# cmusphinx/pocketsphinx

Hardware: NVIDIA H100
Metric: frames/sec senone-eval+Viterbi (higher is better)
Workload: dtype f32->i16/i32

## Files before the change

### pocketsphinx_b200/csrc/psb_hmm.cu

```cuda
#include "psb_hmmctx.cuh"

#include <stdlib.h>
#include <string.h>

#include <algorithm>
#include <type_traits>

#include <vector>


struct psb_phoneloop_s {
    psb_hmmctx_t *c;
    int n_phones, window, beam, pbeam, pip;
    double penalty_weight;
    Stream stream;
    DevBuf<int32_t> d_ssid, d_tmatid;
    DevBuf<uint16_t> d_senid;
};

namespace {

__device__ __forceinline__ void load_hmm(const psb_hmm_t *p, HmmReg &h, int n)
{
#pragma unroll
// ... 283 lines not shown
        if (rc) return rc;
    }
    int rc = ensure_hmm_cap(c, n);
    if (rc) return rc;
    memcpy(c->h_hmms, hmms, (size_t)n * sizeof(psb_hmm_t));
    rc = eval_staged(c, n, senscr, best);
    if (rc) return rc;
    for (int i = 0; i < n; ++i) {
        void *ctx = hmms[i].ctx;
        hmms[i] = c->h_hmms[i];
        hmms[i].ctx = ctx;
    }
    return PSB_OK;
}

extern "C" int psb_hmm_vit_eval_ptrs(psb_hmmctx_t *c, psb_hmm_t *const *hmms, int32_t n, const int16_t *senscr,
                                     int32_t *best)
{
    PSB_REQUIRE(c && n >= 0 && (n == 0 || (hmms && senscr)), "psb_hmm_vit_eval_ptrs: bad argument");
    if (best) *best = PSB_WORST_SCORE;
    if (n == 0) return PSB_OK;
    PSB_CUDA(cudaSetDevice(c->device));
    int rc = ensure_hmm_cap(c, n);
    if (rc) return rc;
    for (int i = 0; i < n; ++i) {
        PSB_REQUIRE(hmms[i], "hmms[%d] is null", i);
        rc = validate_hmm(c, hmms[i], i);
        if (rc) return rc;
        c->h_hmms[i] = *hmms[i];
    }
    rc = eval_staged(c, n, senscr, best);
    if (rc) return rc;
    for (int i = 0; i < n; ++i) {
        void *ctx = hmms[i]->ctx;
        *hmms[i] = c->h_hmms[i];
        hmms[i]->ctx = ctx;
    }
    return PSB_OK;
}


extern "C" int psb_phoneloop_create(psb_hmmctx_t *c, int32_t n_phones, const int32_t *ssid, const int32_t *tmatid,
                                    int32_t window, int32_t beam, int32_t pbeam, int32_t pip, double penalty_weight,
                                    psb_phoneloop_t **out)
{
    PSB_REQUIRE(c && out && n_phones > 0 && ssid && tmatid && window >= 0, "psb_phoneloop_create: bad argument");
    PSB_CUDA(cudaSetDevice(c->device));
    std::vector<uint16_t> senid((size_t)c->n_emit * n_phones);
    int rc = ctx_senids(c, "psb_phoneloop_create", n_phones, ssid, tmatid, senid.data(), 1, n_phones);
    if (rc) return rc;
    std::unique_ptr<psb_phoneloop_t> p(new psb_phoneloop_t());
    p->c = c; p->n_phones = n_phones; p->window = window; p->beam = beam; p->pbeam = pbeam; p->pip = pip;
    p->penalty_weight = penalty_weight;
    rc = p->d_senid.reserve(senid.size());
    if (!rc) rc = p->d_tmatid.reserve((size_t)n_phones);
    if (!rc) rc = p->d_ssid.reserve((size_t)n_phones);
    if (rc) return rc;
    cudaError_t e = cudaMemcpy(p->d_senid, senid.data(), senid.size() * 2, cudaMemcpyHostToDevice);
    if (e == cudaSuccess) e = cudaMemcpy(p->d_tmatid, tmatid, (size_t)n_phones * 4, cudaMemcpyHostToDevice);
    if (e == cudaSuccess) e = cudaMemcpy(p->d_ssid, ssid, (size_t)n_phones * 4, cudaMemcpyHostToDevice);
    if (e == cudaSuccess) e = p->stream.create();
    if (e != cudaSuccess) {
        psb_set_error("psb_phoneloop_create: %s", cudaGetErrorString(e));
        return PSB_ERR_CUDA;
    }
    *out = p.release();
    return PSB_OK;
}

extern "C" void psb_phoneloop_free(psb_phoneloop_t *p)
{
    if (!p) return;
    cudaSetDevice(p->c->device);
    cudaStreamSynchronize(p->stream);
    delete p;
}

int psb_phoneloop_launch(psb_phoneloop_t *p, const int16_t *d_senscr, const int32_t *d_utt_off, int32_t n_utt,
                         int32_t *d_best, int32_t *d_pen, psb_hmm_t *d_final, psb_hmm_t *d_trace, cudaStream_t st)
{
    const int H = p->n_phones, N = p->c->n_emit;
    size_t smem = ((size_t)(2 * N + 4 + p->window) * H + 64) * sizeof(int);
    PSB_REQUIRE(smem <= 227 * 1024, "phone loop with %d HMMs needs %zu bytes of shared memory (max 227 KB)", H, smem);
    PSB_CUDA(cudaFuncSetAttribute(phoneloop_kernel, cudaFuncAttributeMaxDynamicSharedMemorySize, (int)smem));
    int threads = std::min(1024, roundup(H, 32));
    PlParams P;
    P.n_phones = H; P.window = p->window; P.beam = p->beam; P.pbeam = p->pbeam; P.pip = p->pip;
    P.penalty_weight = p->penalty_weight;
    phoneloop_kernel<<<n_utt, threads, smem, st>>>(d_senscr, d_utt_off, dev_ctx(p->c), P, p->d_senid, p->d_tmatid, p->d_ssid,
                                                   d_best, d_pen, d_final, d_trace);
    PSB_LAUNCH_CHECK();
    return PSB_OK;
}

int psb_phoneloop_n_phones(const psb_phoneloop_t *p) { return p->n_phones; }

extern "C" int psb_phoneloop_run_device(psb_phoneloop_t *p, const int16_t *d_senscr, const int32_t *utt_off,
                                        int32_t n_utt, int32_t *d_best, int32_t *d_pen, psb_hmm_t *final_hmms,
                                        void *batch)
{
    PSB_REQUIRE(p && d_senscr && utt_off && n_utt >= 0, "psb_phoneloop_run_device: bad argument");
    if (n_utt == 0) return PSB_OK;
    int rc = ctx_check_utts("psb_phoneloop_run_device", utt_off, n_utt, d_senscr);
    if (rc) return rc;
    PSB_CUDA(cudaSetDevice(p->c->device));
    cudaStream_t st = batch ? psb_batch_stream((psb_batch_t *)batch) : p->stream;
    DevBuf<int32_t> d_off;
    DevBuf<psb_hmm_t> d_final;
    if ((rc = d_off.reserve((size_t)n_utt + 1))) return rc;
    if (final_hmms && (rc = d_final.reserve((size_t)n_utt * p->n_phones))) return rc;
    PSB_CUDA(cudaMemcpyAsync(d_off, utt_off, (size_t)(n_utt + 1) * 4, cudaMemcpyHostToDevice, st));
    rc = psb_phoneloop_launch(p, d_senscr, d_off, n_utt, d_best, d_pen, d_final, nullptr, st);
    if (!rc && final_hmms) {
        cudaError_t e = cudaMemcpyAsync(final_hmms, d_final, (size_t)n_utt * p->n_phones * sizeof(psb_hmm_t),
                                        cudaMemcpyDeviceToHost, st);
        if (e != cudaSuccess) { psb_set_error("%s", cudaGetErrorString(e)); rc = PSB_ERR_CUDA; }
    }
    cudaStreamSynchronize(st);
    return rc;
}

extern "C" int psb_phoneloop_run_host(psb_phoneloop_t *p, const int16_t *senscr, const int32_t *utt_off, int32_t n_utt,
                                      int32_t *best, int32_t *pen, psb_hmm_t *hmm_trace)
{
    PSB_REQUIRE(p && senscr && utt_off && n_utt >= 0, "psb_phoneloop_run_host: bad argument");
    if (n_utt == 0) return PSB_OK;
    int rc = ctx_check_utts("psb_phoneloop_run_host", utt_off, n_utt, senscr);
    if (rc) return rc;
    PSB_CUDA(cudaSetDevice(p->c->device));
    const size_t total = utt_off[n_utt], H = p->n_phones;
    DevBuf<int16_t> d_scr;
    DevBuf<int32_t> d_off, d_best, d_pen;
    DevBuf<psb_hmm_t> d_tr;
    if ((rc = d_scr.reserve(std::max<size_t>(1, total * p->c->n_sen))) || (rc = d_off.reserve((size_t)n_utt + 1)) ||
        (best && (rc = d_best.reserve(std::max<size_t>(1, total)))) || (pen && (rc = d_pen.reserve(std::max<size_t>(1, total * H)))) ||
        (hmm_trace && (rc = d_tr.reserve(std::max<size_t>(1, total * H)))))
        return rc;
    cudaError_t e = cudaMemcpy(d_scr, senscr, total * p->c->n_sen * 2, cudaMemcpyHostToDevice);
    if (e == cudaSuccess) e = cudaMemcpy(d_off, utt_off, (size_t)(n_utt + 1) * 4, cudaMemcpyHostToDevice);
    if (e == cudaSuccess) {
        rc = psb_phoneloop_launch(p, d_scr, d_off, n_utt, d_best, d_pen, nullptr, d_tr, p->stream);
        if (!rc) e = cudaStreamSynchronize(p->stream);
        if (!rc && e == cudaSuccess && best) e = cudaMemcpy(best, d_best, total * 4, cudaMemcpyDeviceToHost);
        if (!rc && e == cudaSuccess && pen) e = cudaMemcpy(pen, d_pen, total * H * 4, cudaMemcpyDeviceToHost);
        if (!rc && e == cudaSuccess && hmm_trace)
            e = cudaMemcpy(hmm_trace, d_tr, total * H * sizeof(psb_hmm_t), cudaMemcpyDeviceToHost);
    }
    if (e != cudaSuccess) { psb_set_error("psb_phoneloop_run_host: %s", cudaGetErrorString(e)); rc = PSB_ERR_CUDA; }
    return rc;
}

constexpr int HS_V = 4;
constexpr int HS_TS = 512;
constexpr int SWEEP_FR = 4;
constexpr int HS_THREADS = 128;

struct psb_hmmset_s {
    psb_hmmctx_t *c;
    int64_t n_max, n, pitch;
    int32_t n_seg_max, n_seg;
    int64_t max_seg_len;
    bool any_mpx;
    Stream own_stream;
    cudaStream_t stream;
    DevBuf<int32_t> d_i32;
    DevBuf<uint16_t> d_u16;
    DevBuf<uint8_t> d_mpx;
    DevBuf<int64_t> d_seg_off;
    DevBuf<int64_t> d_seg_base;
    DevBuf<psb_hmm_t> d_aos;
    DevBuf<int32_t> d_snap_i32;
    Event ev[2];
};

namespace {

struct HmmSetDev {
    int32_t *i32;
    uint16_t *u16;
    uint8_t *mpx;
    const int64_t *seg_off, *seg_base;
    int64_t pitch;
    int n_seg;
};

static HmmSetDev dev_set(const psb_hmmset_t *s)
{
    HmmSetDev d;
    d.i32 = s->d_i32; d.u16 = s->d_u16; d.mpx = s->d_mpx; d.seg_off = s->d_seg_off; d.seg_base = s->d_seg_base;
    d.pitch = s->pitch; d.n_seg = s->n_seg;
    return d;
}

template <bool TO_SOA>
__global__ void __launch_bounds__(256)
hmmset_convert_kernel(psb_hmm_t *aos, HmmSetDev s, int64_t n, int ns)
{
    const int64_t a = (int64_t)blockIdx.x * blockDim.x + threadIdx.x;
    if (a >= n) return;
    int lo = 0, hi = s.n_seg;
    while (hi - lo > 1) {
        const int mid = (lo + hi) >> 1;
        if (s.seg_off[mid] <= a) lo = mid; else hi = mid;
    }
    const int64_t i = s.seg_base[lo] + (a - s.seg_off[lo]);
    psb_hmm_t *p = aos + a;
    const int64_t b32 = (i / HS_TS) * (int64_t)(2 * ns + 4) * HS_TS + (i % HS_TS);
    const int64_t b16 = (i / HS_TS) * (int64_t)(ns + 2) * HS_TS + (i % HS_TS);
    int32_t *score = s.i32 + b32, *hist = score + ns * HS_TS, *tail = score + 2 * ns * HS_TS;
    uint16_t *senid = s.u16 + b16, *ids = senid + ns * HS_TS;
    if (TO_SOA) {
        for (int k = 0; k < ns; ++k) {
            score[k * HS_TS] = p->score[k];
            hist[k * HS_TS] = p->history[k];
            senid[k * HS_TS] = p->senid[k];
        }
        tail[0] = p->out_score; tail[HS_TS] = p->out_history; tail[2 * HS_TS] = p->bestscore; tail[3 * HS_TS] = p->frame;
        ids[0] = p->ssid; ids[HS_TS] = (uint16_t)p->tmatid;
        s.mpx[i] = p->mpx;
    }
    else {
        for (int k = 0; k < PSB_HMM_MAX_NSTATE; ++k) {
            p->score[k] = k < ns ? score[k * HS_TS] : 0;
            p->history[k] = k < ns ? hist[k * HS_TS] : 0;
            p->senid[k] = k < ns ? senid[k * HS_TS] : 0;
        }
        p->out_score = tail[0]; p->out_history = tail[HS_TS]; p->bestscore = tail[2 * HS_TS]; p->frame = tail[3 * HS_TS];
        p->ssid = ids[0]; p->tmatid = (int16_t)ids[HS_TS];
        p->mpx = s.mpx[i]; p->n_emit_state = (uint8_t)ns;
        p->ctx = nullptr;
    }
}

__global__ void fill_i32_kernel(int32_t *p, int64_t n, int32_t v)
{
    const int64_t i = (int64_t)blockIdx.x * blockDim.x + threadIdx.x;
    if (i < n) p[i] = v;
}

__device__ __forceinline__ int comp(const int4 &v, int q) { return q == 0 ? v.x : q == 1 ? v.y : q == 2 ? v.z : v.w; }
__device__ __forceinline__ void setc(int4 &v, int q, int x)
{
    if (q == 0) v.x = x; else if (q == 1) v.y = x; else if (q == 2) v.z = x; else v.w = x;
}

__device__ __forceinline__ void mbar_init(uint64_t *bar, int count)
{
    asm volatile("mbarrier.init.shared::cta.b64 [%0], %1;" ::"r"((unsigned)__cvta_generic_to_shared(bar)), "r"(count));
}
__device__ __forceinline__ void mbar_expect_tx(uint64_t *bar, unsigned bytes)
{
    asm volatile("mbarrier.arrive.expect_tx.shared::cta.b64 _, [%0], %1;" ::"r"((unsigned)__cvta_generic_to_shared(bar)), "r"(bytes)
                 : "memory");
}
__device__ __forceinline__ void mbar_wait(uint64_t *bar, unsigned parity)
{
    asm volatile(
        "{\n"
        ".reg .pred p;\n"
        "WAIT_%=:\n"
        "mbarrier.try_wait.parity.shared::cta.b64 p, [%0], %1;\n"
        "@p bra DONE_%=;\n"
        "bra WAIT_%=;\n"
        "DONE_%=:\n"
        "}\n" ::"r"((unsigned)__cvta_generic_to_shared(bar)),
        "r"(parity)
        : "memory");
}
__device__ __forceinline__ void tma_bulk_g2s(void *dst, const void *src, unsigned bytes, uint64_t *bar)
{
    asm volatile("cp.async.bulk.shared::cluster.global.mbarrier::complete_tx::bytes [%0], [%1], %2, [%3];" ::"r"(
                     (unsigned)__cvta_generic_to_shared(dst)),
                 "l"(src), "r"(bytes), "r"((unsigned)__cvta_generic_to_shared(bar))
                 : "memory");
}

template <int NS>
__global__ void __launch_bounds__(HS_THREADS, NS == 3 ? 6 : 4)
hmmset_eval_kernel(HmmSetDev s, HmmCtxDev c, const int16_t *__restrict__ senscr, const int64_t *__restrict__ row0,
                   const int32_t *__restrict__ n_rows, int t, int32_t *__restrict__ best_out)
{
    extern __shared__ __align__(16) int16_t srow[];
    __shared__ int red[HS_THREADS / 32];
    const int seg = blockIdx.y;
    if (n_rows && t >= n_rows[seg]) return;
    const int64_t n = s.seg_off[seg + 1] - s.seg_off[seg];
    const int64_t j0 = ((int64_t)blockIdx.x * HS_THREADS + threadIdx.x) * HS_V;
    if ((int64_t)blockIdx.x * HS_THREADS * HS_V >= n) return;
    constexpr int NL = NS > 0 ? NS : PSB_HMM_MAX_NSTATE;
    const int ns = NS > 0 ? NS : c.n_emit;
    const bool live = j0 < n;
    const int64_t i = s.seg_base[seg] + (live ? j0 : 0);
    const int64_t b32 = (i / HS_TS) * (int64_t)(2 * ns + 4) * HS_TS + (i % HS_TS);
    const int64_t b16 = (i / HS_TS) * (int64_t)(ns + 2) * HS_TS + (i % HS_TS);
    int32_t *score = s.i32 + b32, *hist = score + ns * HS_TS, *tail = score + 2 * ns * HS_TS;
    uint16_t *senid = s.u16 + b16;
    const uint16_t *ids = senid + ns * HS_TS;
    int4 sc[NL], hi[NL], osc, ohi, bst;
    uint2 sid[NL], tm = make_uint2(0u, 0u);
    uchar4 mp = make_uchar4(0, 0, 0, 0);
    if (live) {
#pragma unroll
        for (int k = 0; k < NL; ++k)
            if (k < ns) {
                sc[k] = __ldcs(reinterpret_cast<const int4 *>(score + k * HS_TS));
                hi[k] = __ldcs(reinterpret_cast<const int4 *>(hist + k * HS_TS));
                sid[k] = __ldcs(reinterpret_cast<const uint2 *>(senid + k * HS_TS));
            }
        osc = __ldcs(reinterpret_cast<const int4 *>(tail));
        ohi = __ldcs(reinterpret_cast<const int4 *>(tail + HS_TS));
        tm = __ldcs(reinterpret_cast<const uint2 *>(ids + HS_TS));
        mp = __ldcs(reinterpret_cast<const uchar4 *>(s.mpx + i));
    }
    __shared__ __align__(8) uint64_t row_bar;
    const int16_t *srow_al;
    {
        const int16_t *row = senscr + (row0 ? row0[seg] + t : (int64_t)t * gridDim.y + seg) * c.n_sen;
        const uintptr_t a = reinterpret_cast<uintptr_t>(row);
        const unsigned mis = (unsigned)(a & 15), nbytes = (unsigned)c.n_sen * 2;
        unsigned head = (16 - mis) & 15;
        if (head > nbytes) head = nbytes;
        const unsigned body = (nbytes - head) & ~15u, tail = nbytes - head - body;
        unsigned char *dst = reinterpret_cast<unsigned char *>(srow) + mis;
        if (threadIdx.x == 0) {
            mbar_init(&row_bar, 1);
            asm volatile("fence.mbarrier_init.release.cluster;" ::: "memory");
            if (body) {
                mbar_expect_tx(&row_bar, body);
                tma_bulk_g2s(dst + head, reinterpret_cast<const unsigned char *>(row) + head, body, &row_bar);
            }
        }
        const unsigned hn = head >> 1, tn = tail >> 1;
        if (threadIdx.x < hn) reinterpret_cast<int16_t *>(dst)[threadIdx.x] = row[threadIdx.x];
        if (threadIdx.x >= 32 && threadIdx.x < 32 + tn)
            reinterpret_cast<int16_t *>(dst + head + body)[threadIdx.x - 32] = row[((head + body) >> 1) + threadIdx.x - 32];
        srow_al = reinterpret_cast<const int16_t *>(dst);
        __syncthreads();
        if (body) mbar_wait(&row_bar, 0u);
    }
    int best = PSB_WORST_SCORE;
    if (live) {
        bool any_mpx = false;
#pragma unroll
        for (int q = 0; q < HS_V; ++q) {
            HmmReg h;
#pragma unroll
            for (int k = 0; k < PSB_HMM_MAX_NSTATE; ++k) {
                const bool in = k < NL && k < ns;
                h.score[k] = in ? comp(sc[k < NL ? k : 0], q) : PSB_WORST_SCORE;
                h.hist[k] = in ? comp(hi[k < NL ? k : 0], q) : -1;
                const unsigned w = (q < 2) ? sid[k < NL ? k : 0].x : sid[k < NL ? k : 0].y;
                h.senid[k] = in ? (int)((q & 1) ? (w >> 16) : (w & 0xffffu)) : PSB_BAD_SSID;
            }
            h.out_score = comp(osc, q);
            h.out_hist = comp(ohi, q);
            h.best = PSB_WORST_SCORE;
            const unsigned tw = (q < 2) ? tm.x : tm.y;
            const int tmatid = (int16_t)((q & 1) ? (tw >> 16) : (tw & 0xffffu));
// ... 194 lines not shown
            if (NS == 3) {
                int (&s3)[3] = *reinterpret_cast<int (*)[3]>(sc[v]);
                int (&h3)[3] = *reinterpret_cast<int (*)[3]>(hi[v]);
                bb = hmm_step_3st_dec<decltype(s1_known)::value>(s3, h3, osc[v], ohi[v], tk[v], score_at(sid[v][0]), score_at(sid[v][1]),
                                      score_at(sid[v][NS > 2 ? 2 : 0]));
            }
            else {
                HmmReg h;
                int obs[PSB_HMM_MAX_NSTATE];
#pragma unroll
                for (int k = 0; k < PSB_HMM_MAX_NSTATE; ++k) {
                    h.score[k] = k < NS ? sc[v][k < NS ? k : 0] : PSB_WORST_SCORE;
                    h.hist[k] = k < NS ? hi[v][k < NS ? k : 0] : -1;
                    h.senid[k] = 0;
                    obs[k] = k < NS ? -score_at(sid[v][k < NS ? k : 0]) : 0;
                }
                h.out_score = osc[v]; h.out_hist = ohi[v]; h.best = PSB_WORST_SCORE;
                bb = hmm_step_5st(h, tps + tmo[v], obs);
#pragma unroll
                for (int k = 0; k < NS; ++k) { sc[v][k] = h.score[k]; hi[v][k] = h.hist[k]; }
                osc[v] = h.out_score; ohi[v] = h.out_hist;
            }
            if (!LIVE_TEST || v * THREADS < rem) best = max(best, bb);
            best_final[v] = bb;
        }
        };
        if (NS == 3 && FAST && s1_live) frame_steps(std::true_type());
        else frame_steps(std::false_type());
        best = __reduce_max_sync(0xffffffffu, best);
        if (BEAM) cnt = __reduce_add_sync(0xffffffffu, cnt);
        const int slot = t % (2 * FR);
        if ((tid & 31) == 0) {
            red[slot][tid >> 5] = best;
            if (BEAM) redc[b][tid >> 5] = cnt;
        }
        if (FR > 1 && t % FR != FR - 1 && t + 1 < T) continue;
        const int tf = t - t % FR;
        __syncthreads();
        if (tid == 0 && !cta_empty)
#pragma unroll 1
            for (int u = tf + NBUF; u <= t + NBUF; ++u)
                if (u < T && tma_ok(u)) issue(u);
        if (tid < 32) {
            if (!BEAM) {
#pragma unroll 1
                for (int u = tf; u <= t; ++u) {
                    int v = tid < THREADS / 32 ? red[u % (2 * FR)][tid] : PSB_WORST_SCORE;
                    v = __reduce_max_sync(0xffffffffu, v);
                    if (tid == 0) atomicMax(best_out + (size_t)u * gridDim.y + seg, v);
                }
            }
            else {
                int v = tid < THREADS / 32 ? red[slot][tid] : PSB_WORST_SCORE;
                v = __reduce_max_sync(0xffffffffu, v);
                int cc = tid < THREADS / 32 ? redc[b][tid] : 0;
                cc = __reduce_add_sync(0xffffffffu, cc);
                if (tid == 0) mbar_expect_tx(&xbar[b], n_rank * 8u);
                if ((unsigned)tid < n_rank)
                    st_async_v2(mapa_shared(&cl_slot[b][my_rank], (unsigned)tid), (unsigned)v, (unsigned)cc,
                                mapa_shared(&xbar[b], (unsigned)tid));
            }
        }
        if (BEAM) {
            mbar_wait(&xbar[b], (unsigned)(t >> 1) & 1u);
            int seg_best = PSB_WORST_SCORE, seg_cnt = 0;
            for (unsigned r = 0; r < n_rank; ++r) {
                const int2 m = cl_slot[b][r];
                seg_best = max(seg_best, m.x);
                seg_cnt += m.y;
            }
            if (my_rank == 0 && tid == 0) {
                best_out[(size_t)t * gridDim.y + seg] = seg_best;
                if (n_active_out) n_active_out[(size_t)t * gridDim.y + seg] = seg_cnt;
            }
            hist[b ^ 1][tid] = 0u;
            int dyn = beam;
            if (maxhmmpf >= 0 && seg_cnt > maxhmmpf) {
                const int bw = -beam / 256;
#pragma unroll
                for (int v = 0; v < V; ++v)
                    if (act[v]) {
                        int bin = (seg_best - best_final[v]) / bw;
                        bin = bin > 255 ? 255 : bin;
                        atomicAdd(&hist[b][bin], 1u);
                    }
                if (tid == 0) found = 256;
                cluster_sync_all();
                unsigned tot = 0;
                for (unsigned r = 0; r < n_rank; ++r) tot += ld_cluster_u32(mapa_shared(&hist[b][tid], r));
                unsigned incl = tot;
#pragma unroll
                for (int o = 1; o < 32; o <<= 1) {
                    const unsigned y = __shfl_up_sync(0xffffffffu, incl, o);
                    if ((tid & 31) >= o) incl += y;
                }
                if ((tid & 31) == 31) scan_w[tid >> 5] = incl;
                __syncthreads();
                for (int w = 0; w < (tid >> 5); ++w) incl += scan_w[w];
                if (incl > (unsigned)maxhmmpf) atomicMin(&found, tid);
                __syncthreads();
                dyn = -(found * bw);
            }
            const int thresh = seg_best + dyn;
#pragma unroll
            for (int v = 0; v < V; ++v)
                if (act[v] && !(best_final[v] > thresh)) {
#pragma unroll
                    for (int k = 0; k < NS; ++k) { sc[v][k] = PSB_WORST_SCORE; hi[v][k] = -1; }
                    osc[v] = PSB_WORST_SCORE; ohi[v] = -1; best_final[v] = PSB_WORST_SCORE;
                    act[v] = false;
                }
        }
    }
    if (BEAM) cluster_sync_all();
#pragma unroll
    for (int v = 0; v < V; ++v) {
        if (!live[v] || !touched[v]) continue;
        int32_t *p32 = state_i32(v);
#pragma unroll
        for (int k = 0; k < NS; ++k) {
            p32[k * HS_TS] = sc[v][k];
            p32[(NS + k) * HS_TS] = hi[v][k];
        }
        p32[2 * NS * HS_TS] = osc[v];
        p32[(2 * NS + 1) * HS_TS] = ohi[v];
        p32[(2 * NS + 2) * HS_TS] = best_final[v];
        if (BEAM) p32[(2 * NS + 3) * HS_TS] = act[v] ? frame0 + T : -1;
    }
}

}

extern "C" void psb_hmmset_free(psb_hmmset_t *s)
{
    if (!s) return;
    cudaSetDevice(s->c->device);
    if (s->stream) cudaStreamSynchronize(s->stream);
    delete s;
}

extern "C" int psb_hmmset_create(psb_hmmctx_t *c, int64_t n_max, int32_t n_seg_max, psb_hmmset_t **out)
{
    PSB_REQUIRE(c && out && n_max > 0 && n_seg_max > 0 && n_seg_max <= 65535, "psb_hmmset_create: bad argument");
    const char *v = getenv("PSB_HMMSET_THREADS");
    PSB_REQUIRE(!v || !strcmp(v, "128"), "psb_hmmset_create: PSB_HMMSET_THREADS=%s; the only accepted value is 128", v);
    PSB_CUDA(cudaSetDevice(c->device));
    std::unique_ptr<psb_hmmset_t> s(new psb_hmmset_t());
    s->c = c; s->n_max = n_max; s->n_seg_max = n_seg_max;
    s->pitch = ((n_max + (int64_t)(HS_V - 1) * n_seg_max + HS_TS - 1) / HS_TS) * HS_TS;
    const int ns = c->n_emit;
    int rc = s->d_i32.reserve((size_t)(2 * ns + 4) * s->pitch);
    if (!rc) rc = s->d_u16.reserve((size_t)(ns + 2) * s->pitch);
    if (!rc) rc = s->d_mpx.reserve((size_t)s->pitch);
    if (!rc) rc = s->d_seg_off.reserve((size_t)n_seg_max + 1);
    if (!rc) rc = s->d_seg_base.reserve((size_t)n_seg_max + 1);
    if (rc) return rc;
    cudaError_t e = s->own_stream.create();
    s->stream = s->own_stream;
    if (e == cudaSuccess) e = s->ev[0].create();
    if (e == cudaSuccess) e = s->ev[1].create();
    if (e != cudaSuccess) {
        psb_set_error("psb_hmmset_create: %s", cudaGetErrorString(e));
        return PSB_ERR_CUDA;
    }
    *out = s.release();
    return PSB_OK;
}

extern "C" int psb_hmmset_use_batch_stream(psb_hmmset_t *s, psb_batch_t *b)
{
    PSB_REQUIRE(s, "psb_hmmset_use_batch_stream: null set");
    PSB_CUDA(cudaStreamSynchronize(s->stream));
    s->stream = b ? psb_batch_stream(b) : s->own_stream;
    return PSB_OK;
}

extern "C" int psb_hmmset_snapshot(psb_hmmset_t *s)
{
    PSB_REQUIRE(s && !s->any_mpx, "psb_hmmset_snapshot: null set or multiplexed instances");
    PSB_CUDA(cudaSetDevice(s->c->device));
    const size_t nb = (size_t)(2 * s->c->n_emit + 4) * s->pitch * 4;
    const int rc = s->d_snap_i32.reserve(nb / 4);
    if (rc) return rc;
    PSB_CUDA(cudaMemcpyAsync(s->d_snap_i32, s->d_i32, nb, cudaMemcpyDeviceToDevice, s->stream));
    return PSB_OK;
}

extern "C" int psb_hmmset_restore(psb_hmmset_t *s)
{
    PSB_REQUIRE(s && s->d_snap_i32, "psb_hmmset_restore: no snapshot");
    PSB_CUDA(cudaSetDevice(s->c->device));
    PSB_CUDA(cudaMemcpyAsync(s->d_i32, s->d_snap_i32, (size_t)(2 * s->c->n_emit + 4) * s->pitch * 4, cudaMemcpyDeviceToDevice, s->stream));
    return PSB_OK;
}

static int hmmset_staging(psb_hmmset_t *s)
{
    return s->d_aos.reserve((size_t)s->n_max);
}

extern "C" int psb_hmmset_upload(psb_hmmset_t *s, const psb_hmm_t *hmms, int64_t n, const int64_t *seg_off, int32_t n_seg)
{
    PSB_REQUIRE(s && n >= 0 && n <= s->n_max && n_seg > 0 && n_seg <= s->n_seg_max && seg_off && (n == 0 || hmms),
                "psb_hmmset_upload: bad argument");
    PSB_REQUIRE(seg_off[0] == 0 && seg_off[n_seg] == n, "psb_hmmset_upload: seg_off must run from 0 to n");
    PSB_CUDA(cudaSetDevice(s->c->device));
    int64_t mx = 0;
    std::vector<int64_t> base((size_t)n_seg + 1);
    base[0] = 0;
    for (int pass = 0; pass < 2; ++pass) {
        const int big = pass == 0 ? HS_TS : HS_V;
        for (int i = 0; i < n_seg; ++i) {
            PSB_REQUIRE(seg_off[i + 1] >= seg_off[i], "psb_hmmset_upload: seg_off not monotone at %d", i);
            const int64_t len = seg_off[i + 1] - seg_off[i];
            const int pad = len >= HS_TS ? big : HS_V;
            mx = std::max<int64_t>(mx, len);
            base[(size_t)i + 1] = base[(size_t)i] + (len + pad - 1) / pad * pad;
        }
        if (base[(size_t)n_seg] <= s->pitch) break;
    }
    PSB_REQUIRE(base[(size_t)n_seg] <= s->pitch, "psb_hmmset_upload: internal capacity exceeded");
    s->any_mpx = false;
    for (int64_t i = 0; i < n; ++i) {
        int rc = validate_hmm(s->c, &hmms[i], (int)i);
        if (rc) return rc;
        s->any_mpx |= hmms[i].mpx != 0;
    }
    int rc = hmmset_staging(s);
    if (rc) return rc;
    s->n = n; s->n_seg = n_seg; s->max_seg_len = mx;
    PSB_CUDA(cudaMemcpyAsync(s->d_seg_off, seg_off, (size_t)(n_seg + 1) * 8, cudaMemcpyHostToDevice, s->stream));
    PSB_CUDA(cudaMemcpyAsync(s->d_seg_base, base.data(), (size_t)(n_seg + 1) * 8, cudaMemcpyHostToDevice, s->stream));
    const int ns = s->c->n_emit;
    const int64_t ni = (int64_t)(2 * ns + 4) * s->pitch;
    fill_i32_kernel<<<(unsigned)((ni + 255) / 256), 256, 0, s->stream>>>(s->d_i32, ni, PSB_WORST_SCORE);
    PSB_LAUNCH_CHECK();
    PSB_CUDA(cudaMemsetAsync(s->d_u16, 0, (size_t)(ns + 2) * s->pitch * 2, s->stream));
    PSB_CUDA(cudaMemsetAsync(s->d_mpx, 0, (size_t)s->pitch, s->stream));
    if (n) {
        PSB_CUDA(cudaMemcpyAsync(s->d_aos, hmms, (size_t)n * sizeof(psb_hmm_t), cudaMemcpyHostToDevice, s->stream));
        hmmset_convert_kernel<true><<<(unsigned)((n + 255) / 256), 256, 0, s->stream>>>(s->d_aos, dev_set(s), n, ns);
        PSB_LAUNCH_CHECK();
    }
    PSB_CUDA(cudaStreamSynchronize(s->stream));
    return PSB_OK;
}

extern "C" int psb_hmmset_download(psb_hmmset_t *s, psb_hmm_t *hmms)
{
    PSB_REQUIRE(s && (s->n == 0 || hmms), "psb_hmmset_download: bad argument");
    if (s->n == 0) return PSB_OK;
    PSB_CUDA(cudaSetDevice(s->c->device));
    int rc = hmmset_staging(s);
    if (rc) return rc;
    hmmset_convert_kernel<false><<<(unsigned)((s->n + 255) / 256), 256, 0, s->stream>>>(s->d_aos, dev_set(s), s->n, s->c->n_emit);
    PSB_LAUNCH_CHECK();
    std::vector<psb_hmm_t> tmp((size_t)s->n);
    PSB_CUDA(cudaMemcpyAsync(tmp.data(), s->d_aos, (size_t)s->n * sizeof(psb_hmm_t), cudaMemcpyDeviceToHost, s->stream));
    PSB_CUDA(cudaStreamSynchronize(s->stream));
    for (int64_t i = 0; i < s->n; ++i) {
        void *ctx = hmms[i].ctx;
        hmms[i] = tmp[(size_t)i];
        hmms[i].ctx = ctx;
    }
    return PSB_OK;
}

extern "C" int psb_hmmset_eval_frames_device(psb_hmmset_t *s, const int16_t *d_senscr, const int64_t *d_row0,
                                             const int32_t *d_n_rows, int32_t n_frames, int32_t *d_best, float *ms)
{
    PSB_REQUIRE(s && d_senscr && d_best && n_frames >= 0, "psb_hmmset_eval_frames_device: bad argument");
    if (ms) *ms = 0.f;
    if (n_frames == 0 || s->n_seg == 0) return PSB_OK;
    PSB_CUDA(cudaSetDevice(s->c->device));
    const int64_t nb = (int64_t)n_frames * s->n_seg;
    fill_i32_kernel<<<(unsigned)((nb + 255) / 256), 256, 0, s->stream>>>(d_best, nb, PSB_WORST_SCORE);
    PSB_LAUNCH_CHECK();
    if (s->n == 0) {
        PSB_CUDA(cudaStreamSynchronize(s->stream));
        return PSB_OK;
    }
    const int tile = HS_THREADS * HS_V;
    const dim3 grid((unsigned)((s->max_seg_len + tile - 1) / tile), (unsigned)s->n_seg);
    const HmmSetDev sd = dev_set(s);
    const HmmCtxDev cd = dev_ctx(s->c);
    const size_t smem = (((size_t)cd.n_sen * 2 + 15) & ~(size_t)15) + 16;
    PSB_REQUIRE(smem <= 200 * 1024, "psb_hmmset: %d senones do not fit the shared-memory score row", cd.n_sen);
    auto launch = [&](auto kern, int t, int32_t *best) {
        kern<<<grid, HS_THREADS, smem, s->stream>>>(sd, cd, d_senscr, d_row0, d_n_rows, t, best);
    };
#define PSB_HS_ATTR(NS) PSB_CUDA(cudaFuncSetAttribute(hmmset_eval_kernel<NS>, cudaFuncAttributeMaxDynamicSharedMemorySize, (int)smem))
    if (smem > 48 * 1024) {
        PSB_HS_ATTR(3); PSB_HS_ATTR(5); PSB_HS_ATTR(0);
    }
#undef PSB_HS_ATTR
    PSB_CUDA(cudaEventRecord(s->ev[0], s->stream));
    for (int t = 0; t < n_frames; ++t) {
        int32_t *best = d_best + (size_t)t * s->n_seg;
        if (cd.n_emit == 3) launch(hmmset_eval_kernel<3>, t, best);
        else if (cd.n_emit == 5) launch(hmmset_eval_kernel<5>, t, best);
        else launch(hmmset_eval_kernel<0>, t, best);
        PSB_LAUNCH_CHECK();
    }
    PSB_CUDA(cudaEventRecord(s->ev[1], s->stream));
    PSB_CUDA(cudaStreamSynchronize(s->stream));
    if (ms) PSB_CUDA(cudaEventElapsedTime(ms, s->ev[0], s->ev[1]));
    return PSB_OK;
}

template <int NS, int V, int THREADS, int FR, bool LIVE_TEST = (NS != 3), bool FAST = (NS == 3)>
static int sweep_launch(psb_hmmset_t *s, const int16_t *d_senscr, int64_t rows_total, const int64_t *d_row0,
                        const int32_t *d_n_rows, int32_t n_frames, int32_t *d_best)
{
    const HmmCtxDev cd = dev_ctx(s->c);
    const int buf_bytes = (int)(((size_t)cd.n_sen * 2 + 32 + 127) & ~(size_t)127);
    const int tp_bytes = s->c->n_tmat * NS * (NS + 1);
    const size_t smem = 2 * FR * (size_t)buf_bytes + tp_bytes;
    PSB_REQUIRE(smem <= 200 * 1024, "psb_hmmset_sweep: %d senones / %d transition matrices do not fit shared memory", cd.n_sen, s->c->n_tmat);
    auto kern = hmmset_sweep_kernel<NS, V, THREADS, false, FR, LIVE_TEST, FAST>;
    PSB_CUDA(cudaFuncSetAttribute(kern, cudaFuncAttributeMaxDynamicSharedMemorySize, (int)smem));
    const dim3 grid((unsigned)((s->max_seg_len + THREADS * V - 1) / (THREADS * V)), (unsigned)s->n_seg);
    PSB_CUDA(cudaEventRecord(s->ev[0], s->stream));
    kern<<<grid, THREADS, smem, s->stream>>>(dev_set(s), cd, d_senscr, (long long)rows_total, d_row0, d_n_rows, n_frames, d_best,
                                            s->c->n_tmat, buf_bytes, 0, 0, -1, nullptr);
    PSB_LAUNCH_CHECK();
    PSB_CUDA(cudaEventRecord(s->ev[1], s->stream));
    return PSB_OK;
}

static int sweep_device(psb_hmmset_t *s, const int16_t *d_senscr, int64_t rows_total, const int64_t *d_row0,
                        const int32_t *d_n_rows, int32_t n_frames, int32_t *d_best, int candidate, float *ms)
{
    PSB_REQUIRE(s && d_senscr && d_best && n_frames >= 0 && rows_total > 0, "psb_hmmset_sweep_device: bad argument");
    const HmmCtxDev cd = dev_ctx(s->c);
    if (s->any_mpx || (cd.n_emit != 3 && cd.n_emit != 5) || (cd.n_sen & 1))
        return psb_hmmset_eval_frames_device(s, d_senscr, d_row0, d_n_rows, n_frames, d_best, ms);
    if (ms) *ms = 0.f;
    if (n_frames == 0 || s->n_seg == 0) return PSB_OK;
    PSB_CUDA(cudaSetDevice(s->c->device));
    const int64_t nb = (int64_t)n_frames * s->n_seg;
    fill_i32_kernel<<<(unsigned)((nb + 255) / 256), 256, 0, s->stream>>>(d_best, nb, PSB_WORST_SCORE);
    PSB_LAUNCH_CHECK();
    if (s->n == 0) {
        if (ms) PSB_CUDA(cudaStreamSynchronize(s->stream));
        return PSB_OK;
    }
    int rc;
    if (cd.n_emit == 5) rc = sweep_launch<5, 4, 512, SWEEP_FR>(s, d_senscr, rows_total, d_row0, d_n_rows, n_frames, d_best);
#ifdef PSB_SWEEP_CANDIDATES
    else if (candidate == 1) rc = sweep_launch<3, 4, 256, 2>(s, d_senscr, rows_total, d_row0, d_n_rows, n_frames, d_best);
    else if (candidate == 2) rc = sweep_launch<3, 4, 512, 1>(s, d_senscr, rows_total, d_row0, d_n_rows, n_frames, d_best);
    else if (candidate == 3) rc = sweep_launch<3, 4, 512, 4, false, false>(s, d_senscr, rows_total, d_row0, d_n_rows, n_frames, d_best);
    else if (candidate == 4) rc = sweep_launch<3, 4, 512, 8>(s, d_senscr, rows_total, d_row0, d_n_rows, n_frames, d_best);
    else if (candidate == 5) rc = sweep_launch<3, 4, 256, 2, true, false>(s, d_senscr, rows_total, d_row0, d_n_rows, n_frames, d_best);
    else if (candidate == 6) rc = sweep_launch<3, 4, 512, 2, true, false>(s, d_senscr, rows_total, d_row0, d_n_rows, n_frames, d_best);
    else if (candidate == 7) rc = sweep_launch<3, 4, 512, 2>(s, d_senscr, rows_total, d_row0, d_n_rows, n_frames, d_best);
    else if (candidate == 8) rc = sweep_launch<3, 4, 256, 4>(s, d_senscr, rows_total, d_row0, d_n_rows, n_frames, d_best);
#endif
    else rc = sweep_launch<3, 4, 512, SWEEP_FR>(s, d_senscr, rows_total, d_row0, d_n_rows, n_frames, d_best);
    (void)candidate;
    if (rc) return rc;
    if (ms) {
        PSB_CUDA(cudaStreamSynchronize(s->stream));
        PSB_CUDA(cudaEventElapsedTime(ms, s->ev[0], s->ev[1]));
    }
    return PSB_OK;
}

extern "C" int psb_hmmset_sweep_device(psb_hmmset_t *s, const int16_t *d_senscr, int64_t rows_total, const int64_t *d_row0,
                                       const int32_t *d_n_rows, int32_t n_frames, int32_t *d_best, float *ms)
{
    return sweep_device(s, d_senscr, rows_total, d_row0, d_n_rows, n_frames, d_best, 0, ms);
}

#ifdef PSB_SWEEP_CANDIDATES
extern "C" int psb_hmmset_sweep_candidate_device(psb_hmmset_t *s, const int16_t *d_senscr, int64_t rows_total, const int64_t *d_row0,
                                                 const int32_t *d_n_rows, int32_t n_frames, int32_t *d_best, int32_t candidate,
                                                 float *ms)
{
    return sweep_device(s, d_senscr, rows_total, d_row0, d_n_rows, n_frames, d_best, candidate, ms);
}
#endif

extern "C" int psb_hmmset_sweep_beam_device(psb_hmmset_t *s, const int16_t *d_senscr, int64_t rows_total, const int64_t *d_row0,
                                            const int32_t *d_n_rows, int32_t n_frames, int32_t frame0, int32_t beam,
                                            int32_t maxhmmpf, int32_t *d_best, int32_t *d_n_active, float *ms)
{
    PSB_REQUIRE(s && d_senscr && d_best && n_frames >= 0 && rows_total > 0, "psb_hmmset_sweep_beam_device: bad argument");
    PSB_REQUIRE(beam < 0 && beam > -0x20000000, "psb_hmmset_sweep_beam_device: the beam is a negative log score (got %d)", beam);
    PSB_REQUIRE(maxhmmpf < 0 || beam <= -256, "psb_hmmset_sweep_beam_device: -maxhmmpf needs a beam of at least 256 score units (bin width -beam/256)");
    const HmmCtxDev cd = dev_ctx(s->c);
    PSB_REQUIRE(!s->any_mpx && (cd.n_emit == 3 || cd.n_emit == 5) && !(cd.n_sen & 1),
                "psb_hmmset_sweep_beam_device: plain 3- or 5-state instances and an even senone count (the fused kernel's shapes)");
    constexpr int THREADS = 256, V = 4;
    const int64_t per_seg = (s->max_seg_len + THREADS * V - 1) / (THREADS * V);
    PSB_REQUIRE(per_seg <= 16, "psb_hmmset_sweep_beam_device: a segment of %lld instances needs %lld CTAs, a cluster holds 16",
                (long long)s->max_seg_len, (long long)per_seg);
    if (ms) *ms = 0.f;
    if (n_frames == 0 || s->n_seg == 0) return PSB_OK;
    PSB_CUDA(cudaSetDevice(s->c->device));
    const int64_t nb = (int64_t)n_frames * s->n_seg;
    fill_i32_kernel<<<(unsigned)((nb + 255) / 256), 256, 0, s->stream>>>(d_best, nb, PSB_WORST_SCORE);
    PSB_LAUNCH_CHECK();
    if (d_n_active) PSB_CUDA(cudaMemsetAsync(d_n_active, 0, (size_t)nb * 4, s->stream));
    if (s->n == 0) {
        if (ms) PSB_CUDA(cudaStreamSynchronize(s->stream));
        return PSB_OK;
    }
    const int buf_bytes = (int)(((size_t)cd.n_sen * 2 + 32 + 127) & ~(size_t)127);
    const int tp_bytes = s->c->n_tmat * cd.n_emit * (cd.n_emit + 1);
    const size_t smem = 6 * (size_t)buf_bytes + tp_bytes;
    PSB_REQUIRE(smem <= 200 * 1024, "psb_hmmset_sweep_beam: %d senones / %d transition matrices do not fit shared memory", cd.n_sen, s->c->n_tmat);
    const HmmSetDev sd = dev_set(s);
    const long long rows_ll = rows_total;
    const int n_tmat = s->c->n_tmat;
    cudaLaunchConfig_t cfg = {};
    cfg.gridDim = dim3((unsigned)std::max<int64_t>(per_seg, 1), (unsigned)s->n_seg);
    cfg.blockDim = dim3(THREADS);
    cfg.dynamicSmemBytes = smem;
    cfg.stream = s->stream;
    cudaLaunchAttribute at[1];
    at[0].id = cudaLaunchAttributeClusterDimension;
    at[0].val.clusterDim.x = cfg.gridDim.x; at[0].val.clusterDim.y = 1; at[0].val.clusterDim.z = 1;
    cfg.attrs = at; cfg.numAttrs = 1;
    PSB_CUDA(cudaEventRecord(s->ev[0], s->stream));
#define PSB_SWEEPB(NS)                                                                                                         \
    do {                                                                                                                       \
        auto kern = hmmset_sweep_kernel<NS, V, THREADS, true>;                                                                 \
        PSB_CUDA(cudaFuncSetAttribute(kern, cudaFuncAttributeMaxDynamicSharedMemorySize, (int)smem));                          \
        if (cfg.gridDim.x > 8) PSB_CUDA(cudaFuncSetAttribute(kern, cudaFuncAttributeNonPortableClusterSizeAllowed, 1));       \
        int n_clusters = 0;                                                                                                    \
        PSB_CUDA(cudaOccupancyMaxActiveClusters(&n_clusters, kern, &cfg));                                                     \
        PSB_REQUIRE(n_clusters > 0, "psb_hmmset_sweep_beam: a cluster of %u CTAs with %zu bytes of shared memory each does not fit the device", \
                    cfg.gridDim.x, smem);                                                                                      \
        PSB_CUDA(cudaLaunchKernelEx(&cfg, kern, sd, cd, d_senscr, rows_ll, d_row0, d_n_rows, (int)n_frames, d_best, n_tmat,   \
                                    buf_bytes, (int)frame0, (int)beam, (int)maxhmmpf, d_n_active));                            \
        PSB_LAUNCH_CHECK();                                                                                                    \
    } while (0)
    if (cd.n_emit == 3) PSB_SWEEPB(3);
    else PSB_SWEEPB(5);
#undef PSB_SWEEPB
    PSB_CUDA(cudaEventRecord(s->ev[1], s->stream));
    if (ms) {
        PSB_CUDA(cudaStreamSynchronize(s->stream));
        PSB_CUDA(cudaEventElapsedTime(ms, s->ev[0], s->ev[1]));
    }
    return PSB_OK;
}

extern "C" int psb_hmmset_eval_host(psb_hmmset_t *s, const int16_t *senscr, int32_t *best)
{
    PSB_REQUIRE(s && senscr && best, "psb_hmmset_eval_host: bad argument");
    PSB_CUDA(cudaSetDevice(s->c->device));
    DevBuf<int16_t> d_scr;
    DevBuf<int32_t> d_best;
    const size_t nb = (size_t)s->n_seg * s->c->n_sen * 2;
    int rc = d_scr.reserve(nb / 2);
    if (!rc) rc = d_best.reserve((size_t)s->n_seg);
    if (rc) return rc;
    cudaError_t e = cudaMemcpy(d_scr, senscr, nb, cudaMemcpyHostToDevice);
    if (e == cudaSuccess) {
        rc = psb_hmmset_eval_frames_device(s, d_scr, nullptr, nullptr, 1, d_best, nullptr);
        if (!rc) e = cudaMemcpy(best, d_best, (size_t)s->n_seg * 4, cudaMemcpyDeviceToHost);
    }
    if (e != cudaSuccess) {
        psb_set_error("psb_hmmset_eval_host: %s", cudaGetErrorString(e));
        return PSB_ERR_CUDA;
    }
    return rc;
}

namespace {

__global__ void __launch_bounds__(128)
align_kernel(const int16_t *__restrict__ senscr, const int32_t *__restrict__ utt_off, HmmCtxDev c,
             const int32_t *__restrict__ ph_off, const uint16_t *__restrict__ senid_g,
             const int32_t *__restrict__ tmatid_g, const int32_t *__restrict__ sf_g, const int32_t *__restrict__ ef_g,
             int32_t *__restrict__ tok_id, int32_t *__restrict__ tok_sc, const int64_t *__restrict__ tok_row,
             const int32_t *__restrict__ band_lo, const int32_t *__restrict__ band_hi,
             int32_t *__restrict__ st_start, int32_t *__restrict__ st_dur, int32_t *__restrict__ st_score,
             int32_t *__restrict__ status)
{
    extern __shared__ int sm[];
    const int u = blockIdx.x, tid = threadIdx.x, N = c.n_emit;
    const int p0 = ph_off[u], H = ph_off[u + 1] - p0;
    const long long f0 = utt_off[u];
    const int T = utt_off[u + 1] - utt_off[u];
    const int n_st = H * N;
    int *score = sm;
    int *hist = score + N * H;
    int *out_score = hist + N * H;
    int *out_hist = out_score + H;
    int *frame = out_hist + H;
    int *sval = frame + H;
    int *sidx = sval + 32;
    const HmmSoA<false> V{score, hist, out_score, out_hist, nullptr, H};
    const int64_t *row_u = tok_row + f0;
    const int32_t *lo_u = band_lo + f0, *hi_u = band_hi + f0;
    int32_t *ss = st_start + (size_t)p0 * N, *sd = st_dur + (size_t)p0 * N, *sc = st_score + (size_t)p0 * N;

    for (int i = tid; i < n_st; i += blockDim.x) { ss[i] = -1; sd[i] = -1; sc[i] = -1; }
    if (H == 0) { if (tid == 0) status[u] = -1; return; }
    for (int i = tid; i < H; i += blockDim.x) {
        V.clear(i, N);
        frame[i] = -1;
    }
    __syncthreads();
    if (tid == 0) { score[0] = 0; hist[0] = 0; frame[0] = 0; }
    int best_score = 0;
    __syncthreads();

    for (int t = 0; t < T; ++t) {
// ... 779 lines not shown
```

Before: 12.73 million.

## Sort HMMs by first senone within each CTA slice and widen sweep frame batch

Measured after the change: 12.83 million, median of 6. Within noise of the previous version (+0.8%).

```diff
diff --git a/pocketsphinx_b200/csrc/psb_hmm.cu b/pocketsphinx_b200/csrc/psb_hmm.cu
--- a/pocketsphinx_b200/csrc/psb_hmm.cu
+++ b/pocketsphinx_b200/csrc/psb_hmm.cu
@@ -459,7 +459,8 @@
 
 constexpr int HS_V = 4;
 constexpr int HS_TS = 512;
-constexpr int SWEEP_FR = 4;
+constexpr int SWEEP_FR = 4, SWEEP_FR_WIDE = 8;
+constexpr int SWEEP_SLICE = 512 * 4;
 constexpr int HS_THREADS = 128;
 
 struct psb_hmmset_s {
@@ -473,6 +474,7 @@
     DevBuf<int32_t> d_i32;
     DevBuf<uint16_t> d_u16;
     DevBuf<uint8_t> d_mpx;
+    DevBuf<uint16_t> d_slot;
     DevBuf<int64_t> d_seg_off;
     DevBuf<int64_t> d_seg_base;
     DevBuf<psb_hmm_t> d_aos;
@@ -501,7 +503,7 @@
 
 template <bool TO_SOA>
 __global__ void __launch_bounds__(256)
-hmmset_convert_kernel(psb_hmm_t *aos, HmmSetDev s, int64_t n, int ns)
+hmmset_convert_kernel(psb_hmm_t *aos, HmmSetDev s, const uint16_t *__restrict__ slot, int64_t n, int ns)
 {
     const int64_t a = (int64_t)blockIdx.x * blockDim.x + threadIdx.x;
     if (a >= n) return;
@@ -510,7 +512,8 @@
         const int mid = (lo + hi) >> 1;
         if (s.seg_off[mid] <= a) lo = mid; else hi = mid;
     }
-    const int64_t i = s.seg_base[lo] + (a - s.seg_off[lo]);
+    const int64_t r = a - s.seg_off[lo];
+    const int64_t i = s.seg_base[lo] + (r - r % SWEEP_SLICE) + slot[a];
     psb_hmm_t *p = aos + a;
     const int64_t b32 = (i / HS_TS) * (int64_t)(2 * ns + 4) * HS_TS + (i % HS_TS);
     const int64_t b16 = (i / HS_TS) * (int64_t)(ns + 2) * HS_TS + (i % HS_TS);
@@ -1011,6 +1014,7 @@
     int rc = s->d_i32.reserve((size_t)(2 * ns + 4) * s->pitch);
     if (!rc) rc = s->d_u16.reserve((size_t)(ns + 2) * s->pitch);
     if (!rc) rc = s->d_mpx.reserve((size_t)s->pitch);
+    if (!rc) rc = s->d_slot.reserve((size_t)n_max);
     if (!rc) rc = s->d_seg_off.reserve((size_t)n_seg_max + 1);
     if (!rc) rc = s->d_seg_base.reserve((size_t)n_seg_max + 1);
     if (rc) return rc;
@@ -1056,6 +1060,21 @@
 static int hmmset_staging(psb_hmmset_t *s)
 {
     return s->d_aos.reserve((size_t)s->n_max);
+}
+
+static std::vector<uint16_t> slot_order(const psb_hmm_t *hmms, const int64_t *seg_off, int32_t n_seg)
+{
+    static_assert(SWEEP_SLICE <= 65536, "places are uint16");
+    std::vector<uint16_t> slot((size_t)seg_off[n_seg]);
+    std::vector<uint32_t> key(SWEEP_SLICE);
+    for (int i = 0; i < n_seg; ++i)
+        for (int64_t a = seg_off[i]; a < seg_off[i + 1]; a += SWEEP_SLICE) {
+            const int m = (int)std::min<int64_t>(SWEEP_SLICE, seg_off[i + 1] - a);
+            for (int k = 0; k < m; ++k) key[(size_t)k] = (uint32_t)hmms[a + k].senid[0] << 16 | (uint32_t)k;
+            std::sort(key.begin(), key.begin() + m);
+            for (int q = 0; q < m; ++q) slot[(size_t)(a + (key[(size_t)q] & 0xffffu))] = (uint16_t)q;
+        }
+    return slot;
 }
 
 extern "C" int psb_hmmset_upload(psb_hmmset_t *s, const psb_hmm_t *hmms, int64_t n, const int64_t *seg_off, int32_t n_seg)
@@ -1097,8 +1116,10 @@
     PSB_CUDA(cudaMemsetAsync(s->d_u16, 0, (size_t)(ns + 2) * s->pitch * 2, s->stream));
     PSB_CUDA(cudaMemsetAsync(s->d_mpx, 0, (size_t)s->pitch, s->stream));
     if (n) {
+        const std::vector<uint16_t> slot = slot_order(hmms, seg_off, n_seg);
+        PSB_CUDA(cudaMemcpyAsync(s->d_slot, slot.data(), slot.size() * 2, cudaMemcpyHostToDevice, s->stream));
         PSB_CUDA(cudaMemcpyAsync(s->d_aos, hmms, (size_t)n * sizeof(psb_hmm_t), cudaMemcpyHostToDevice, s->stream));
-        hmmset_convert_kernel<true><<<(unsigned)((n + 255) / 256), 256, 0, s->stream>>>(s->d_aos, dev_set(s), n, ns);
+        hmmset_convert_kernel<true><<<(unsigned)((n + 255) / 256), 256, 0, s->stream>>>(s->d_aos, dev_set(s), s->d_slot, n, ns);
         PSB_LAUNCH_CHECK();
     }
     PSB_CUDA(cudaStreamSynchronize(s->stream));
@@ -1112,7 +1133,7 @@
     PSB_CUDA(cudaSetDevice(s->c->device));
     int rc = hmmset_staging(s);
     if (rc) return rc;
-    hmmset_convert_kernel<false><<<(unsigned)((s->n + 255) / 256), 256, 0, s->stream>>>(s->d_aos, dev_set(s), s->n, s->c->n_emit);
+    hmmset_convert_kernel<false><<<(unsigned)((s->n + 255) / 256), 256, 0, s->stream>>>(s->d_aos, dev_set(s), s->d_slot, s->n, s->c->n_emit);
     PSB_LAUNCH_CHECK();
     std::vector<psb_hmm_t> tmp((size_t)s->n);
     PSB_CUDA(cudaMemcpyAsync(tmp.data(), s->d_aos, (size_t)s->n * sizeof(psb_hmm_t), cudaMemcpyDeviceToHost, s->stream));
@@ -1167,15 +1188,21 @@
     return PSB_OK;
 }
 
+static int sweep_buf_bytes(const psb_hmmctx_t *c) { return (int)(((size_t)c->n_sen * 2 + 32 + 127) & ~(size_t)127); }
+static size_t sweep_smem(const psb_hmmctx_t *c, int n_buf)
+{
+    return n_buf * (size_t)sweep_buf_bytes(c) + (size_t)c->n_tmat * c->n_emit * (c->n_emit + 1);
+}
+constexpr size_t SWEEP_SMEM_MAX = 200 * 1024;
+
 template <int NS, int V, int THREADS, int FR, bool LIVE_TEST = (NS != 3), bool FAST = (NS == 3)>
 static int sweep_launch(psb_hmmset_t *s, const int16_t *d_senscr, int64_t rows_total, const int64_t *d_row0,
                         const int32_t *d_n_rows, int32_t n_frames, int32_t *d_best)
 {
     const HmmCtxDev cd = dev_ctx(s->c);
-    const int buf_bytes = (int)(((size_t)cd.n_sen * 2 + 32 + 127) & ~(size_t)127);
-    const int tp_bytes = s->c->n_tmat * NS * (NS + 1);
-    const size_t smem = 2 * FR * (size_t)buf_bytes + tp_bytes;
-    PSB_REQUIRE(smem <= 200 * 1024, "psb_hmmset_sweep: %d senones / %d transition matrices do not fit shared memory", cd.n_sen, s->c->n_tmat);
+    const int buf_bytes = sweep_buf_bytes(s->c);
+    const size_t smem = sweep_smem(s->c, 2 * FR);
+    PSB_REQUIRE(smem <= SWEEP_SMEM_MAX, "psb_hmmset_sweep: %d senones / %d transition matrices do not fit shared memory", cd.n_sen, s->c->n_tmat);
     auto kern = hmmset_sweep_kernel<NS, V, THREADS, false, FR, LIVE_TEST, FAST>;
     PSB_CUDA(cudaFuncSetAttribute(kern, cudaFuncAttributeMaxDynamicSharedMemorySize, (int)smem));
     const dim3 grid((unsigned)((s->max_seg_len + THREADS * V - 1) / (THREADS * V)), (unsigned)s->n_seg);
@@ -1205,18 +1232,15 @@
         return PSB_OK;
     }
     int rc;
-    if (cd.n_emit == 5) rc = sweep_launch<5, 4, 512, SWEEP_FR>(s, d_senscr, rows_total, d_row0, d_n_rows, n_frames, d_best);
+    static_assert(512 * 4 == SWEEP_SLICE, "the slice that upload orders is one CTA's");
+    const bool wide = sweep_smem(s->c, 2 * SWEEP_FR_WIDE) <= SWEEP_SMEM_MAX;
+#define PSB_SWEEP_ARGS s, d_senscr, rows_total, d_row0, d_n_rows, n_frames, d_best
+    if (cd.n_emit == 5) rc = wide ? sweep_launch<5, 4, 512, SWEEP_FR_WIDE>(PSB_SWEEP_ARGS) : sweep_launch<5, 4, 512, SWEEP_FR>(PSB_SWEEP_ARGS);
 #ifdef PSB_SWEEP_CANDIDATES
-    else if (candidate == 1) rc = sweep_launch<3, 4, 256, 2>(s, d_senscr, rows_total, d_row0, d_n_rows, n_frames, d_best);
-    else if (candidate == 2) rc = sweep_launch<3, 4, 512, 1>(s, d_senscr, rows_total, d_row0, d_n_rows, n_frames, d_best);
-    else if (candidate == 3) rc = sweep_launch<3, 4, 512, 4, false, false>(s, d_senscr, rows_total, d_row0, d_n_rows, n_frames, d_best);
-    else if (candidate == 4) rc = sweep_launch<3, 4, 512, 8>(s, d_senscr, rows_total, d_row0, d_n_rows, n_frames, d_best);
-    else if (candidate == 5) rc = sweep_launch<3, 4, 256, 2, true, false>(s, d_senscr, rows_total, d_row0, d_n_rows, n_frames, d_best);
-    else if (candidate == 6) rc = sweep_launch<3, 4, 512, 2, true, false>(s, d_senscr, rows_total, d_row0, d_n_rows, n_frames, d_best);
-    else if (candidate == 7) rc = sweep_launch<3, 4, 512, 2>(s, d_senscr, rows_total, d_row0, d_n_rows, n_frames, d_best);
-    else if (candidate == 8) rc = sweep_launch<3, 4, 256, 4>(s, d_senscr, rows_total, d_row0, d_n_rows, n_frames, d_best);
+    else if (candidate == 1) rc = sweep_launch<3, 4, 512, SWEEP_FR>(PSB_SWEEP_ARGS);
 #endif
-    else rc = sweep_launch<3, 4, 512, SWEEP_FR>(s, d_senscr, rows_total, d_row0, d_n_rows, n_frames, d_best);
+    else rc = wide ? sweep_launch<3, 4, 512, SWEEP_FR_WIDE>(PSB_SWEEP_ARGS) : sweep_launch<3, 4, 512, SWEEP_FR>(PSB_SWEEP_ARGS);
+#undef PSB_SWEEP_ARGS
     (void)candidate;
     if (rc) return rc;
     if (ms) {
```
